# codelibs/ranklib

Measured on AMD Instinct MI355X. Metric: boosting rounds/sec (LambdaMART -ranker 6, NDCG@10), higher is better.
Workload: dtype int64 fixed-point histograms + f64 lambdas/scores (f32 leaf chains as in the Java)

## Files before the change

ranklib_amd/_native.py:

```python
import ctypes as C
import os

import numpy as np

_HERE = os.path.dirname(os.path.abspath(__file__))
LIB_PATH = os.environ.get("RLHIP_LIB") or os.path.join(_HERE, "lib", "librlhip.so")


class RankLibError(RuntimeError):
    """Mirrors ciir.umass.edu.utilities.RankLibError (utilities/RankLibError.java:9-43)."""


class RlParams(C.Structure):
    _fields_ = [("n_trees", C.c_int32), ("n_leaves", C.c_int32), ("n_threshold", C.c_int32),
                ("min_leaf_support", C.c_int32), ("early_stop_rounds", C.c_int32), ("learning_rate", C.c_float),
                ("metric", C.c_int32), ("metric_k", C.c_int32), ("device", C.c_int32), ("flags", C.c_int32),
                ("ranker", C.c_int32), ("feature_sampling_rate", C.c_float), ("seed", C.c_uint64)]


RL_METRIC = dict(NDCG=0, DCG=1, MAP=2, ERR=3, P=4, RR=5)
RL_CA_METRIC = dict(NDCG=0, DCG=1, MAP=2, ERR=3, P=4, RR=5)
RL_NORM_KIND = dict(sum=0, zscore=1, linear=2)
RL_EVAL_METRIC = dict(RL_CA_METRIC, BEST=6)

# ... 581 lines not shown
        need = C.c_int64(0)
        check(lib().rl_model_to_text(self.h, None, 0, C.byref(need)))
        buf = C.create_string_buffer(need.value)
        check(lib().rl_model_to_text(self.h, buf, need.value, C.byref(need)))
        return buf.value.decode("ascii")

    def bin_stride(self):
        s = C.c_int32(0)
        check(lib().rl_bin_stride(self.h, C.byref(s)))
        return s.value

    def quant_exponent(self):
        e = C.c_int32(0)
        check(lib().rl_quant_exponent(self.h, C.byref(e)))
        return e.value

    def hist_features(self):
        n = C.c_int32(0)
        check(lib().rl_hist_features(self.h, C.byref(n), None, 0))
        cols = np.zeros(n.value, np.int32)
        check(lib().rl_hist_features(self.h, C.byref(n), cols.ctypes.data_as(C.POINTER(C.c_int32)), n.value))
        return n.value, cols

    def array(self, name):
        which = ARR[name]
        TS = self.bin_stride()
        F_hist = self.hist_features()[0] if name in ("NBINS", "THRESHOLDS", "BINS", "ROOT_COUNT", "ROOT_SUM", "ROOT_SUM_FIXED", "ROOT_SUM_JAVA") else self.F
        shapes = {
            "LAMBDA": ((self.N,), np.float64), "WEIGHT": ((self.N,), np.float64), "SCORE": ((self.N,), np.float64),
            "VALID_SCORE": ((self.Nv,), np.float64), "NBINS": ((F_hist,), np.int32),
            "THRESHOLDS": ((F_hist, TS), np.float32), "BINS": ((F_hist, self.N), np.uint16),
            "ROOT_COUNT": ((F_hist, TS), np.int32), "ROOT_SUM": ((F_hist, TS), np.float64), "ROOT_SUM_JAVA": ((F_hist, TS), np.float64),
            "QUANT": ((self.N,), np.int64), "ROOT_SUM_FIXED": ((F_hist, TS, 2), np.int64),
            "NDCG_PER_QUERY": ((self.Q,), np.float64), "CHAIN_STATS": ((6,), np.int32), "GROW_STATS": ((4,), np.int32), "GROW_DOCS": ((4,), np.int64), "BUBBLES": ((4,), np.int64), "PIECE_STATS": ((2,), np.int64), "SPARSE_INFO": ((8,), np.int64), "PHASE_CLOCKS": ((64, 32), np.int64), "BLOCK_TRACE": ((64, 3, 2048, 8), np.int64), "STEP_LOG": ((8 + 8 * 8192,), np.int32), "TIE_STATS": ((10,), np.int64), "LAUNCH_ARMS": ((ARM["COUNT_"],), np.int64), "CHAIN_MISS": ((2, self.cap + 1), np.int32),
        }
        shape, dt = shapes[name]
        out = np.zeros(shape, dt)
        check(lib().rl_get_array(self.h, which, out.ctypes.data, out.nbytes))
        return out

    def timing(self, kernel):
        ms, n, b = C.c_double(0), C.c_int64(0), C.c_double(0)
        check(lib().rl_get_timing(self.h, KERNEL[kernel], C.byref(ms), C.byref(n), C.byref(b)))
        return ms.value, n.value, b.value

    def reset_timing(self):
        check(lib().rl_reset_timing(self.h))

    def set_timing_flags(self, flags):
        check(lib().rl_set_timing_flags(self.h, flags))

    def close(self):
        if getattr(self, "h", None) and self.h.value:
            lib().rl_destroy(self.h)
            self.h = C.c_void_p()

    def __del__(self):
        try:
            self.close()
        except Exception:
            pass


MODEL_PATH_NONE, MODEL_PATH_TILED, MODEL_PATH_GENERIC = 0, 1, 2
MODEL_PATH_PERMUTED = 3
PERMUTED_BATCH = 16
MODEL_PATH_COVER, MODEL_PATH_CONTRIBS = 4, 5
# ... 630 lines not shown
```

ranklib_amd/csrc/rl_internal.h:

```cpp
#pragma once
#include <hip/hip_runtime.h>
#include <stdint.h>

#include <string>
#include <vector>

#include "../../include/rlhip.h"

namespace rl {

constexpr int kThreads = 256;
constexpr int kWave = 64;
constexpr int kFinThreads = 320;
constexpr int kLog2Chunk = 14;
constexpr int kChunk = 1 << kLog2Chunk;
#ifndef RL_NODE_CHUNK
#define RL_NODE_CHUNK 8192
#endif
constexpr int kNodeChunk = RL_NODE_CHUNK;
constexpr int kMinChunk = 512;
#ifndef RL_HIST_DOCS
#define RL_HIST_DOCS 2
#endif
constexpr int kHistDocs = RL_HIST_DOCS;
// ... 34 lines not shown
    double  sq_response;
    long long tot_hi; unsigned long long tot_lo;
    long long sq;
    float   output; int32_t gcount;
    int32_t pl, pr;
    int32_t fid;
    int32_t prepared;
    int32_t best_cl, tie;
    unsigned long long ph;
    long long best_hi; unsigned long long best_lo;
};

struct SlotRec {
    int32_t node, left, right, build_left;
    int32_t pstart, pcount, pbuf, f, t;
    int32_t tile0, ntiles;
    int32_t chunk0, nchunks;
    int32_t nleft;
    int32_t cs, skip_hist;
    long long sq_left;
};

struct TreeState {
    int32_t n_nodes, nslots, done, taken;
    int32_t qsize, n_leaves, E, E2;
    int32_t n_splits, error, tiles_total, chunks_total;
    int32_t arrive, epoch, step, tree_seq;
    unsigned long long maxabs_bits;
    long long root_sq;
    int32_t stall_n, stall_node[kSpec], defer_any, stall_pad[2 + (4 - kSpec % 4) % 4];
    SlotRec slot[kSpec];
    int32_t arrive1[kSpec][16];
};

struct TreeSlot {
    int32_t n_nodes, pad;
};

struct FeatBest;
struct Ctx {
    int32_t N, Npad, Q, F, TS, L, MAXN, NC, mls, k, maxChunks, nTiles, FG, numFG;
    float lr;
    int32_t rank, n_ranks;
    int32_t sharded;
    int32_t Nglobal;
    int32_t sub_child;
    int32_t hist_nt;
    int32_t node_div, node_min, node_chunk;
    const int32_t *live_nthr;
    int32_t n_live; const int32_t *live;
    int32_t limb_words;
    const int32_t *fcol;
    int32_t fs_on;
    int32_t fs_size;
    unsigned long long seed;
    int32_t tie_on;
    int32_t mart, metric;
    long long *dist_buf;
    const uint16_t *bins;
    const uint16_t *gbins;
    const uint16_t *dbins;
    int32_t p8, pd_stride;
    const unsigned char *pbins;
    const uint16_t *phib;
    const unsigned char *pdbins;
    const uint8_t *cr_grp;
// ... 108 lines not shown
```

ranklib_amd/csrc/rl_k_ensemble.inc:

```

namespace rl {

struct EnsTree {
    int32_t *feat_idx;
    float *thr;
    int32_t *left, *right;
    float *out;
    int32_t *n_nodes;
    int32_t *count;
    double *deviance;
};

__global__ __launch_bounds__(kThreads) void k_export_tree(const Ctx c, const EnsTree e, int tree)
{
    const TreeState *st = c.st;
    const int nn = st->n_nodes;
    for (int i = threadIdx.x; i < nn; i += kThreads) {
        const NodeRec &X = c.nodes[i];
        if (X.fid < 0) continue;
        const size_t o = (size_t)tree * c.MAXN + X.fid;
        const bool leaf = X.left < 0;
        e.feat_idx[o] = leaf ? -1 : (c.vcol ? c.vcol[X.best_f] : X.best_f);
        e.thr[o] = leaf ? 0.f : c.thr[(size_t)X.best_f * c.TS + X.best_t];
        e.left[o] = leaf ? -1 : c.nodes[X.left].fid; e.right[o] = leaf ? -1 : c.nodes[X.right].fid;
        e.out[o] = leaf ? X.output : 0.f;
        e.count[o] = X.gcount;
        e.deviance[o] = X.deviance;
    }
    if (threadIdx.x == 0) e.n_nodes[tree] = 2 * st->n_splits + 1;
}

__global__ __launch_bounds__(kThreads) void k_valid_update(const EnsTree e, int MAXN, int tree, const float *X, int n, int F,
                                                            float lr, double *vscores)
{
    const size_t o = (size_t)tree * MAXN;
    for (int i = blockIdx.x * kThreads + threadIdx.x; i < n; i += gridDim.x * kThreads) {
        const float *row = X + (size_t)i * F;
        int nd = 0;
        while (e.feat_idx[o + nd] != -1) nd = (row[e.feat_idx[o + nd]] <= e.thr[o + nd]) ? e.left[o + nd] : e.right[o + nd];
        vscores[i] += (double)lr * (double)e.out[o + nd];
    }
}

__global__ __launch_bounds__(kThreads) void k_ensemble_eval(const EnsTree e, int MAXN, int nt, const float *X, int64_t n,
                                                             int stride, float w, float *out, double *out_d)
{
    for (int64_t i = (int64_t)blockIdx.x * kThreads + threadIdx.x; i < n; i += (int64_t)gridDim.x * kThreads) {
        const float *row = X + (size_t)i * stride;
        float s = 0.f;
        for (int t = 0; t < nt; t++) {
            const size_t o = (size_t)t * MAXN;
            int nd = 0;
            while (e.feat_idx[o + nd] != -1) {
                const int fc = e.feat_idx[o + nd];
                const float v = (fc < stride) ? row[fc] : 0.f;
                nd = (v <= e.thr[o + nd]) ? e.left[o + nd] : e.right[o + nd];
            }
            s = (float)((double)s + (double)e.out[o + nd] * (double)w);
        }
        if (out) out[i] = s;
        if (out_d) out_d[i] = (double)s;
    }
// ... 4 lines not shown
```

ranklib_amd/csrc/rl_k_leaf.inc:

```

namespace rl {

constexpr int kLeafTableCap = 1024;

__global__ __launch_bounds__(kThreads) void k_leaf_table(const Ctx c, const ChainBufs cb, int32_t *seg_buf)
{
    __shared__ int s_left[kLeafTableCap], s_right[kLeafTableCap], s_start[kLeafTableCap], s_buf[kLeafTableCap], s_stack[kLeafTableCap];
    TreeState *st = c.st;
    if (threadIdx.x == 0 && c.grow_docs[8] != 0ull) {
        const unsigned long long now = wall_clock64();
        c.grow_docs[4] += now - c.grow_docs[8]; c.grow_docs[5] += 1ull; c.grow_docs[8] = 0ull;
    }
    const int nn = st->n_nodes;
    if (nn <= kLeafTableCap) {
        for (int x = threadIdx.x; x < nn; x += kThreads) {
            const NodeRec &X = c.nodes[x];
            s_left[x] = X.left; s_right[x] = X.right; s_start[x] = X.start; s_buf[x] = X.buf;
        }
        __syncthreads();
        if (threadIdx.x != 0) return;
        int n = 0, sp = 0, tiles = 0, prev = 0;
        s_stack[sp++] = 0;
        while (sp > 0) {
            const int x = s_stack[--sp];
// ... 106 lines not shown
        for (int p = blockIdx.x * kThreads + threadIdx.x; p < N; p += gridDim.x * kThreads) {
            int lo = 0, hi = nl - 1;
            while (lo < hi) { const int mid = (lo + hi + 1) >> 1; if (c.leaf_start[mid] <= p) lo = mid; else hi = mid - 1; }
            const int node = c.leaf_node[lo];
            const NodeRec &X = c.nodes[node];
            const int k = (node == 0) ? p : c.idx[X.buf][p];
            c.scores[k] += (double)c.lr * (double)X.output;
        }
        return;
    }
    constexpr int RUN = kScoreBatch * kThreads;
    for (int base = blockIdx.x * RUN; base < N; base += gridDim.x * RUN) {
        int p[kScoreBatch], k[kScoreBatch]; double step[kScoreBatch], sc[kScoreBatch];
        int buf[kScoreBatch];
#pragma unroll
        for (int u = 0; u < kScoreBatch; u++) {
            p[u] = min(base + u * kThreads + (int)threadIdx.x, N - 1);
            int lo = 0, hi = nl - 1;
            while (lo < hi) { const int mid = (lo + hi + 1) >> 1; if (s_start[mid] <= p[u]) lo = mid; else hi = mid - 1; }
            buf[u] = s_buf[lo]; step[u] = s_step[lo];
        }
#pragma unroll
        for (int u = 0; u < kScoreBatch; u++) k[u] = c.idx[max(buf[u], 0)][p[u]];
#pragma unroll
        for (int u = 0; u < kScoreBatch; u++) { if (buf[u] < 0) k[u] = p[u]; }
#pragma unroll
        for (int u = 0; u < kScoreBatch; u++) sc[u] = c.scores[k[u]];
#pragma unroll
        for (int u = 0; u < kScoreBatch; u++)
            if (base + u * kThreads + (int)threadIdx.x < N) c.scores[k[u]] = sc[u] + step[u];
    }
}

__global__ __launch_bounds__(kThreads) void k_score_stream(const Ctx c)
{
    __shared__ double s_step[1024];
    const TreeState *st = c.st;
    const int nl = st->n_leaves;
    for (int i = threadIdx.x; i < nl; i += kThreads) s_step[i] = (double)c.lr * (double)c.nodes[c.leaf_node[i]].output;
    __syncthreads();
    const int N = c.N;
    constexpr int RUN = kScoreBatch * kThreads;
    for (int base = blockIdx.x * RUN; base < N; base += gridDim.x * RUN) {
        int k[kScoreBatch]; unsigned short lf[kScoreBatch]; double sc[kScoreBatch];
#pragma unroll
        for (int u = 0; u < kScoreBatch; u++) { k[u] = min(base + u * kThreads + (int)threadIdx.x, N - 1); lf[u] = c.leaf_of[k[u]]; sc[u] = c.scores[k[u]]; }
#pragma unroll
        for (int u = 0; u < kScoreBatch; u++)
            if (base + u * kThreads + (int)threadIdx.x < N) c.scores[k[u]] = sc[u] + s_step[min((int)lf[u], 1023)];
    }
}

__global__ __launch_bounds__(64) void k_float_mean(const double *v, int n, float *out)
{
    float s = 0.f;
    for (int base = 0; base < n; base += 64) {
        const int i = base + lane_id();
        const double x = (i < n) ? v[i] : 0.0;
        const uint32_t a0 = (uint32_t)d2bits(x), a1 = (uint32_t)(d2bits(x) >> 32);
        const int m = min(64, n - base);
#pragma unroll
        for (int j = 0; j < 64; j++) {
            if (j < m) {
                const uint64_t ua = ((uint64_t)(uint32_t)__builtin_amdgcn_readlane((int)a1, j) << 32) | (uint32_t)__builtin_amdgcn_readlane((int)a0, j);
                s = float_chain_step(s, bits2d(ua));
            }
        }
    }
    if (lane_id() == 0) *out = s / (float)n;
}

__global__ __launch_bounds__(64) void k_double_mean(const double *v, int n, double *out)
{
    if (threadIdx.x != 0) return;
    double s = 0.0;
    for (int i = 0; i < n; i++) s += v[i];
    *out = s / n;
}

}
```

ranklib_amd/csrc/rl_k_select.inc:

```

namespace rl {

__device__ __forceinline__ void queue_insert_lds(int *q, double *qd, int &qsize, int node, double d)
{
    int i = 0;
    while (i < qsize) { if (qd[i] > d) i++; else break; }
    for (int j = qsize; j > i; j--) { q[j] = q[j - 1]; qd[j] = qd[j - 1]; }
    q[i] = node; qd[i] = d;
    qsize++;
}

__device__ __forceinline__ int node_chunks(const Ctx &c, int cnt) { return cnt <= 0 ? 0 : (cnt + chunk_docs<false>(c, cnt) - 1) / chunk_docs<false>(c, cnt); }

__device__ __forceinline__ void prepare_children(const Ctx &c, NodeRec *N, int p, int l, SlotRec &sl)
{
    NodeRec &P = N[p];
    const int r = l + 1;
    const int cl = P.best_cl;
    const long long thi = P.best_hi; const unsigned long long tlo = P.best_lo;
    NodeRec Lc, Rc;
    Lc.start = P.start; Lc.count = 0; Lc.gcount = cl; Lc.buf = 1 - P.buf; Lc.parent = p; Lc.left = Lc.right = -1;
    Rc.start = P.start; Rc.count = 0; Rc.gcount = P.gcount - cl; Rc.buf = 1 - P.buf; Rc.parent = p; Rc.left = Rc.right = -1;
    const i128 tl = make_i128(thi, tlo);
    const i128 tr = make_i128(P.tot_hi, P.tot_lo) - tl;
// ... 365 lines not shown
    if (tid < nsel) prepare_children(c, N, sel[tid], nn0 + 2 * tid, st.slot[tid]);
    if (c.steplog && tid < nsel) {
        const int e = atomicAdd(&c.steplog[0], 1);
        if (e < kStepLogCap) {
            int *o = c.steplog + 8 + 8 * e; const NodeRec &P = N[sel[tid]];
            o[0] = st.tree_seq; o[1] = 0; o[2] = st.step + 1; o[3] = tid; o[4] = P.gcount; o[5] = st.slot[tid].build_left ? P.best_cl : P.gcount - P.best_cl; o[6] = P.tie; o[7] = nsel;
        }
    }
    __syncthreads();
    if (tid == 0) {
        int tiles = 0, chunks = 0;
        balance_slots(c, st.slot, nsel);
        for (int j = 0; j < nsel; j++) {
            st.slot[j].tile0 = tiles; tiles += st.slot[j].ntiles;
            st.slot[j].chunk0 = chunks; chunks += st.slot[j].nchunks;
        }
        st.tiles_total = tiles; st.chunks_total = chunks;
        st.n_nodes = nn0 + 2 * nsel;
        st.arrive = 0; st.epoch++;
        for (int j = 0; j < kSpec * 16; j++) (&st.arrive1[0][0])[j] = 0;
    }
    __syncthreads();
    RL_CLK(true, 12);
    if (nodes_in_lds) copy_words(c.nodes, N, st.n_nodes * (int)(sizeof(NodeRec) / 8));
    RL_CLK(true, 13);
#ifdef RL_PHASE_CLOCKS
    if (tid == 0 && st.tree_seq == c.trace_tree) c.clk[(st.step & 63) * 32 + 28] = (long long)wall_clock64();
#endif
    if (tid == 0) st.step++;
    __syncthreads();
    copy_words(c.st, &st, sizeof(TreeState) / 8);
    if (tid == 0 && c.progress)
        __hip_atomic_store(c.progress, ((unsigned long long)(unsigned)st.tree_seq << 32) | (st.stall_n > 0 ? (1ull << 31) : 0ull) | (st.defer_any ? (1ull << 30) : 0ull) |
                                           ((unsigned long long)((unsigned)st.step & 0x1fffffffu) << 1) | (st.done ? 1ull : 0ull),
                           __ATOMIC_RELAXED, __HIP_MEMORY_SCOPE_SYSTEM);
}

template <bool WIDE = false>
__device__ __forceinline__ void select_step(const Ctx &c, bool is_root, unsigned char *smem, bool nodes_in_lds, bool dist)
{
    if (nodes_in_lds) select_step_t<true, WIDE>(c, is_root, smem, dist);
    else select_step_t<false, WIDE>(c, is_root, smem, dist);
}

}
```

ranklib_amd/csrc/rl_round.inc:

```

namespace rl {

struct RoundPlan {
    size_t hist_lds, red_lds, par_lds, fin_lds, slot_words;
    int hist_gx, rootCs, rootChunks, nodes_in_lds, jbg, steps;
};

static int round_plan(const rl_trainer *t, RoundPlan &pl)
{
    const Ctx &c = t->ctx;
    pl.hist_lds = (size_t)c.sub * ((c.sub == 16 && c.TS <= kHistLdsStride) ? kHistLdsStride : c.TS) * 12;
    pl.hist_gx = c.numFG * (kHistFG / c.sub);
    pl.red_lds = (size_t)c.TS * 20;
    pl.rootCs = std::min(kChunk, std::max(kMinChunk, (((c.N + 63) / 64 + 255) & ~255)));
    pl.rootChunks = (c.N + pl.rootCs - 1) / pl.rootCs;
    pl.nodes_in_lds = (select_lds_bytes(c.L, c.NC, true, c.F, c.fs_on != 0) <= 60 * 1024) ? 1 : 0;
    pl.par_lds = (c.TS <= kParCacheTS) ? (size_t)c.TS * 20 + 8 : 0;
    pl.fin_lds = std::max((size_t)c.TS * (c.java ? 28 : 20) + 8 + pl.par_lds, select_lds_bytes(c.L, c.NC, pl.nodes_in_lds != 0, c.F, c.fs_on != 0));
    pl.jbg = (c.TS + 63) / 64;
    if (pl.fin_lds > 128 * 1024) return fail(RL_ERR_UNSUPPORTED, "too many features / leaves for the growth bookkeeping in LDS (feature sampling needs 64 bytes per feature)");
    pl.steps = std::max(c.L - 1, 1);
    pl.slot_words = (size_t)c.F * c.TS * c.limb_words + 4;
    return RL_OK;
}

static int enqueue_lambdas(rl_trainer *t, int &n_max)
{
    Ctx &c = t->ctx;
    hipStream_t s = t->stream;
    const int m = t->round;
    RL_HIP(hipMemsetAsync(&c.st->maxabs_bits, 0, sizeof(unsigned long long) + sizeof(long long), s));
    n_max = 0;
    if (c.mart) {
        ScopedTiming tm(t, RL_KERNEL_LAMBDA, (double)c.N * 20.0);
        n_max = std::min(2048, (c.N + kThreads - 1) / kThreads);
        t->arms[RL_ARM_LAM_MART]++;
        hipLaunchKernelGGL(k_mart_residual, dim3(n_max), dim3(kThreads), 0, s, c.labels, (const double *)c.scores, c.lw, c.N, t->d_wmax);
    } else {
        ScopedTiming tm(t, RL_KERNEL_LAMBDA, (double)c.N * 28.0);
        const double *ideal = (c.metric == RL_METRIC_NDCG) ? (m == 0 ? c.ideal0 : c.ideal1) : nullptr;
        LamArgs g{t->tr.d_ss, t->tr.d_sl, t->tr.d_srel, t->tr.d_sidx, c.qoff, t->tr.d_docq, ideal, c.disc,
                  t->d_T, c.lw, &c.st->maxabs_bits, c.N, c.k, c.k, c.metric, t->p.metric_k,
                  t->tr.d_aux_i, t->tr.d_aux_a, t->tr.d_aux_b, t->d_wmax, t->tr.d_ext_rd};
        if (t->d_T == nullptr) {
            const int mode = (c.metric == RL_METRIC_ERR) ? 1 : (c.metric == RL_METRIC_MAP) ? 2 : (c.metric == RL_METRIC_P) ? 3 : (c.metric == RL_METRIC_RR) ? 4 : 0;
            static const int mode_arm[5] = {RL_ARM_LAM_FUSED, RL_ARM_LAM_ERR, RL_ARM_LAM_MAP, -1, -1};
            const bool cp = t->knobs.lam_compact && mode == 0;
            auto lds_of = [&](int bt) { return (size_t)c.k * (bt + 8) * 16 + (size_t)c.k * 24 + lambda_fused_extra_bytes(mode, c.k, bt) + (cp ? lambda_fused_cp_bytes(c.k, bt) : 0); };
            n_max = 0;
            const DataSet &d = t->tr;
            int lam_used = 0;
            RL_HIP(hipEventRecord(t->ev_lam_fork, s));
            auto lam_stream = [&]() -> hipStream_t {
                const int lam_side = t->knobs.lam_side;
                if (lam_used >= lam_side) return s;
                hipStream_t ls = t->lam_s[lam_used++];
                (void)hipStreamWaitEvent(ls, t->ev_lam_fork, 0);
                return ls;
            };
#define RL_LAUNCH_FUSED(BT, cls)                                                                                                             \
            if (d.n_qcls[cls] > 0) {                                                                                                         \
                hipStream_t ls = lam_stream();                                                                                               \
                if (cp) t->arms[RL_ARM_LAM_COMPACT]++; else if (mode_arm[mode] >= 0) t->arms[mode_arm[mode]]++;                               \
                t->arms[ls == s ? RL_ARM_LAM_ON_MAIN : RL_ARM_LAM_ON_SIDE]++;                                                                \
// ... 59 lines not shown
        if (c.sp_on) {
            hipLaunchKernelGGL(k_hist_sp<kHistLdsStride>, dim3(c.sp_ngroups, pl.rootChunks), dim3(kSpThreads), (size_t)kHistFG * kHistLdsStride * 8, s, c, pl.rootCs);
        }
    }
    if (t->dist) {
        hipLaunchKernelGGL(k_hist_reduce, dim3(c.F), dim3(kFinThreads), pl.red_lds, s, c, 1);
        int rcd = t->dist->allreduce(c.dist_buf, (size_t)c.F * c.TS * c.limb_words + 4, DT_I64, OP_SUM, s);
        if (rcd) return rcd;
        hipLaunchKernelGGL((k_hist_finish<true, true>), dim3(c.F), dim3(kFinThreads), pl.fin_lds, s, c, pl.nodes_in_lds);
    } else if (c.java) {
        hipLaunchKernelGGL(k_jgather, dim3((c.N + kPartTile - 1) / kPartTile), dim3(kThreads), 0, s, c, 1);
        if (c.jmap) hipLaunchKernelGGL(k_jhist2, dim3(c.n_live + 1, 1), dim3(kJ2Threads), 0, s, c, 1, c.jmap, c.jinv, c.jone);
        else hipLaunchKernelGGL(k_jhist, dim3(c.n_live, pl.jbg + 2, 1), dim3(64), 0, s, c, 1, pl.jbg);
        hipLaunchKernelGGL((k_hist_finish<true, false, true>), dim3(c.n_live), dim3(kFinThreads), pl.fin_lds, s, c, pl.nodes_in_lds);
    } else if (t->knobs.step2 && c.TS <= kFin2MaxT) {
        hipLaunchKernelGGL(k_fin2_root, dim3(c.n_live), dim3(kFin2RootThreads), 0, s, c, pl.rootChunks);
        hipLaunchKernelGGL(k_select_root, dim3(1), dim3(kFinThreads), pl.fin_lds, s, c, pl.nodes_in_lds);
    } else hipLaunchKernelGGL((k_hist_finish<true, false>), dim3(c.n_live), dim3(kFinThreads), pl.fin_lds, s, c, pl.nodes_in_lds);
    t->tree_seq++;
    return RL_OK;
}

struct Growth {
    int it = 0, extra = 0;
    bool throttle;
    bool saw_end = false;
    bool defer_seen = false;
    explicit Growth(const Ctx &c) : throttle(c.progress != nullptr) {}
};
enum class Next { Go, Again, Ended };

static bool word_stalled(const rl_trainer *t, unsigned long long w) { return t->ctx.tie_on && (w >> 32) == t->tree_seq && ((w >> 31) & 1ull); }
static bool word_finished(const rl_trainer *t, unsigned long long w) { return (w >> 32) == t->tree_seq && (w & 1); }

static int after_stall(rl_trainer *t, const RoundPlan &pl, Growth &g, Next &next)
{
    Ctx &c = t->ctx;
    int rcs = resolve_ties(t, pl.fin_lds, pl.nodes_in_lds);
    if (rcs) return rcs;
    g.extra += 2;
    bool ended, deferred;
    if (c.progress) {
        const unsigned long long w = __atomic_load_n(t->h_progress, __ATOMIC_ACQUIRE);
        if ((w >> 32) != t->tree_seq) return fail(RL_ERR_STATE, "tie-break: the progress word is not this tree's (internal error)");
        ended = (w & 1ull) != 0;
        deferred = ((w >> 30) & 1ull) != 0;
        g.it = (int)((unsigned)(w & 0x3fffffffull) >> 1);
    } else {
        TreeState sth;
        RL_HIP(hipMemcpy(&sth, c.st, sizeof(sth), hipMemcpyDeviceToHost));
        ended = sth.done != 0;
        deferred = sth.defer_any != 0;
        g.it = sth.step;
    }
    if (ended) g.defer_seen = deferred;
    next = ended ? Next::Ended : Next::Again;
    return RL_OK;
}

static int growth_gate(rl_trainer *t, const RoundPlan &pl, Growth &g, Next &next)
{
    Ctx &c = t->ctx;
    hipStream_t s = t->stream;
    next = Next::Go;
    if (g.throttle && c.tie_on && !t->dist) {
        const unsigned long long w0 = __atomic_load_n(t->h_progress, __ATOMIC_ACQUIRE);
        if (word_stalled(t, w0)) return after_stall(t, pl, g, next);
    }
    const int ahead = t->dist ? t->knobs.dist_ahead : t->knobs.step_ahead;
    if (!g.throttle || g.it < ahead) return RL_OK;
    const unsigned long long want = ((unsigned long long)t->tree_seq << 32) | ((unsigned long long)(unsigned)(g.it - ahead) << 1);
    unsigned long long w = __atomic_load_n(t->h_progress, __ATOMIC_ACQUIRE);
    if (t->dist) {
        unsigned spins = 0;
        const auto t0w = std::chrono::steady_clock::now();
        while ((w & ~(3ull << 30)) < want && !word_finished(t, w) && !word_stalled(t, w)) {
            w = __atomic_load_n(t->h_progress, __ATOMIC_ACQUIRE);
            if ((++spins & 0xfffff) == 0) {
                const hipError_t q = hipStreamQuery(s);
                if (q != hipSuccess && q != hipErrorNotReady) return fail(RL_ERR_HIP, std::string("device error while growing a tree: ") + hipGetErrorString(q));
                if (std::chrono::duration<double>(std::chrono::steady_clock::now() - t0w).count() > t->knobs.dist_timeout_s)
                    return fail(RL_ERR_COMM, "timed out after " + std::to_string((int)t->knobs.dist_timeout_s) + " s waiting for growth step " + std::to_string(g.it - ahead) +
                                             " of tree " + std::to_string(t->tree_seq) + " (a rank of the job is missing from a collective?)");
            }
        }
        const int step_w = (int)((unsigned)(w & 0x3fffffffull) >> 1);
        if (word_finished(t, w) && step_w <= g.it - ahead) { g.defer_seen = ((w >> 30) & 1ull) != 0; next = Next::Ended; return RL_OK; }
        if (word_stalled(t, w) && step_w <= g.it - ahead) return after_stall(t, pl, g, next);
    } else {
        const auto behind = [&](unsigned long long v) {
            if ((v >> 32) != t->tree_seq) return true;
            return (unsigned)((v & 0x3fffffffull) >> 1) < (unsigned)(g.it - ahead) && !(v & 1) && !((v >> 31) & 1);
        };
        if (behind(w)) {
            const auto t0 = std::chrono::steady_clock::now();
            unsigned spins = 0;
            while (behind(w = __atomic_load_n(t->h_progress, __ATOMIC_ACQUIRE))) {
                if ((++spins & 1023) == 0 && std::chrono::steady_clock::now() - t0 > std::chrono::milliseconds(200)) { g.throttle = false; break; }
            }
        }
        if (word_stalled(t, w)) next = Next::Again;
        else if (word_finished(t, w)) { g.defer_seen = ((w >> 30) & 1ull) != 0; next = Next::Ended; }
    }
    return RL_OK;
}

static int enqueue_growth_step(rl_trainer *t, const RoundPlan &pl, Growth &g, Next &next)
{
    Ctx &c = t->ctx;
    hipStream_t s = t->stream;
    next = Next::Go;
    if (t->dist && !c.cum_cnt_loc) {
        hipLaunchKernelGGL(k_part_count, dim3(c.nTiles), dim3(kThreads), 0, s, c);
        hipLaunchKernelGGL(k_part_scatter<false>, dim3(c.nTiles), dim3(kThreads), 0, s, c);
    } else hipLaunchKernelGGL(k_part_scatter<true>, dim3(c.nTiles), dim3(kThreads), 0, s, c);
    t->arms[RL_ARM_STEPS_ENQUEUED]++;
    {
        ScopedTiming tm(t, RL_KERNEL_HIST_NODE, 0.0);
        launch_hist<false>(c, t->knobs, t->arms, pl.hist_gx, c.maxChunks, pl.hist_lds, s);
    }
    if (t->dist) {
        hipLaunchKernelGGL(k_hist_reduce, dim3(c.F, kSpec), dim3(kFinThreads), pl.red_lds, s, c, 0);
        const int max_slots = std::min(kSpec, 1 << std::min(g.it, 8));
        int rcd = t->dist->allreduce(c.dist_buf, pl.slot_words * max_slots, DT_I64, OP_SUM, s);
        if (rcd) return rcd;
        const size_t sel2_lds_d = select2_lds_bytes(c.L, c.NC);
        if (t->knobs.step2 && c.TS <= kFin2MaxT && !c.fs_on && c.F <= kSel2MaxF && c.L > 0 && c.L + 2 <= 64 && sel2_lds_d <= 60 * 1024) {
            hipLaunchKernelGGL(k_fin2<true>, dim3(c.F, kSpec), dim3(kFin2Threads), 0, s, c);
            hipLaunchKernelGGL(k_select2<false>, dim3(1), dim3(kSel2Threads), sel2_lds_d, s, c);
        } else hipLaunchKernelGGL((k_hist_finish<false, true>), dim3(c.F, kSpec), dim3(kFinThreads), pl.fin_lds, s, c, pl.nodes_in_lds);
        if (!c.progress && g.it + 1 < pl.steps + g.extra && ((g.it >= 7 && (g.it - 7) % 3 == 0) || c.tie_on)) {
            TreeState sth;
            RL_HIP(hipStreamSynchronize(s));
            RL_HIP(hipMemcpy(&sth, c.st, sizeof(sth), hipMemcpyDeviceToHost));
            if (sth.stall_n > 0) return after_stall(t, pl, g, next);
// ... 48 lines not shown
    Ctx &c = t->ctx;
    hipStream_t s = t->stream;
    hipLaunchKernelGGL(k_leaf_table, dim3(1), dim3(kThreads), 0, s, c, t->leaf_chain, t->d_seg_buf);
    if (t->p.flags & RL_FLAG_SERIAL_CHAIN) {
        hipLaunchKernelGGL(k_leaf_chain, dim3(c.L), dim3(64), 0, s, c);
        return RL_OK;
    }
    if (t->p.flags & RL_FLAG_FAST_LEAF) {
        const FastLeafArgs fa{c.lw, c.idx[0], c.idx[1], t->d_seg_buf, c.leaf_start, &c.st->n_leaves, c.MAXN + 1, stream_scores ? c.leaf_of : nullptr,
                              t->d_fast_part, (int32_t)t->fast_slots, t->d_fast_sums, c.nodes, c.leaf_node, c.mart};
        hipLaunchKernelGGL(k_fast_leaf_tiles, dim3((unsigned)t->fast_slots), dim3(kFastTile), 0, s, fa);
        hipLaunchKernelGGL(k_fast_leaf_finish, dim3((unsigned)(c.MAXN + 1)), dim3(kFastTile), 0, s, fa);
        return RL_OK;
    }
    const ChainSource src{nullptr, nullptr, c.lw, c.idx[0], c.idx[1], t->d_seg_buf, stream_scores ? c.leaf_of : nullptr};
    const ChainBufs *sums = &t->leaf_chain;
    if (t->dist && t->piece_chains) {
        int rcp = enqueue_leaf_chains_pieces(t, src);
        if (rcp) return rcp;
    } else if (t->dist) {
        int rco = enqueue_leaf_chains_owner(t, src);
        if (rco) return rco;
        sums = &t->gchain;
    } else enqueue_chain(t, t->leaf_chain, src);
    hipLaunchKernelGGL(k_leaf_output, dim3((c.L + kThreads - 1) / kThreads), dim3(kThreads), 0, s, c, *sums);
    return RL_OK;
}

static int enqueue_scores_and_metrics(rl_trainer *t, bool stream_scores)
{
    Ctx &c = t->ctx;
    hipStream_t s = t->stream;
    const int m = t->round;
    if (stream_scores) hipLaunchKernelGGL(k_score_stream, dim3(std::max(1, std::min(2048, (c.N + kScoreBatch * kThreads - 1) / (kScoreBatch * kThreads)))), dim3(kThreads), 0, s, c);
    else hipLaunchKernelGGL(k_score_update, dim3(std::max(1, std::min(4096, (c.N + kScoreBatch * kThreads - 1) / (kScoreBatch * kThreads)))), dim3(kThreads), 0, s, c);
    hipLaunchKernelGGL(k_export_tree, dim3(1), dim3(kThreads), 0, s, c, t->ens, m);
    RL_HIP(hipGetLastError());
    const bool use_side = !t->has_valid;
    if (use_side && t->side_pending) RL_HIP(hipStreamWaitEvent(s, t->ev_metric, 0));
    int rc = launch_rank(t, t->tr, c.scores, t->tr.d_ndcg, true);
    if (rc != RL_OK) return rc;
    if (use_side) {
        const double *mq = t->tr.d_ndcg; int mQ = t->tr.Q;
        if (t->dist) { rc = gather_queries(t, t->tr.d_ndcg, &mq); if (rc != RL_OK) return rc; mQ = t->Qglobal; }
        RL_HIP(hipEventRecord(t->ev_ranked, s));
        RL_HIP(hipStreamWaitEvent(t->side, t->ev_ranked, 0));
        enqueue_metric_mean(t, mq, mQ, c.round_metric + 2 * (size_t)m, t->side);
        RL_HIP(hipEventRecord(t->ev_metric, t->side));
        t->side_pending = true;
    } else if (t->dist) {
        const double *gq = nullptr;
        rc = gather_queries(t, t->tr.d_ndcg, &gq);
        if (rc != RL_OK) return rc;
        enqueue_metric_mean(t, gq, t->Qglobal, c.round_metric + 2 * (size_t)m);
    } else enqueue_metric_mean(t, t->tr.d_ndcg, t->tr.Q, c.round_metric + 2 * (size_t)m);
    if (t->has_valid) {
        hipLaunchKernelGGL(k_valid_update, dim3(std::min<int64_t>(4096, (t->va.N + kThreads - 1) / kThreads)), dim3(kThreads), 0, s,
                           t->ens, c.MAXN, m, (const float *)t->va.d_X, (int)t->va.N, t->F, c.lr, t->va.d_scores);
        rc = launch_rank(t, t->va, t->va.d_scores, t->va.d_ndcg, false);
        if (rc != RL_OK) return rc;
        if (t->dist) {
            const double *gq = nullptr;
            rc = gather_queries(t, t->va.d_ndcg, &gq, true);
            if (rc != RL_OK) return rc;
            enqueue_metric_mean(t, gq, t->vQglobal, c.round_metric + 2 * (size_t)m + 1);
        } else enqueue_metric_mean(t, t->va.d_ndcg, t->va.Q, c.round_metric + 2 * (size_t)m + 1);
    }
    RL_HIP(hipGetLastError());
    t->round = m + 1;
// ... 34 lines not shown
```

ranklib_amd/csrc/rl_step2.inc:

```

namespace rl {

constexpr int kFin2Threads = 320;
constexpr int kFin2Waves = kFin2Threads / 64;
constexpr int kFin2MaxT = kFin2Threads;

struct Fin2WaveRec { double S; int t, c, flags; };

template <bool DIST = false>
__global__ __launch_bounds__(kFin2Threads) void k_fin2(const Ctx c)
{
    const TreeState *st = c.st;
    RL_TR_BEGIN();
    const int slot = blockIdx.y;
    const int st_done = st->done, st_nslots = st->nslots, E = st->E;
    const SlotRec sl = st->slot[slot];
    const int f = (!DIST && c.live) ? c.live[blockIdx.x] : (int)blockIdx.x;
    const int TS = c.TS, T = (!DIST && c.live) ? c.live_nthr[blockIdx.x] : c.nthr[f];
    if (st_done || slot >= st_nslots) return;
    const bool sq_block = blockIdx.x == 0;
    if (sl.skip_hist && !sq_block) return;
    const int tid = threadIdx.x, lane = tid & 63, wave = tid >> 6;
    const int nodeP = sl.node, nodeB = sl.build_left ? sl.left : sl.right, nodeS = sl.build_left ? sl.right : sl.left, sideB = sl.build_left ? 0 : 1;
    const int ch0 = sl.chunk0;
// ... 602 lines not shown
        }
        __builtin_amdgcn_fence(__ATOMIC_ACQ_REL, "workgroup");
        __builtin_amdgcn_wave_barrier();
        if (lane == 0) {
            if (nsel == 1 && budget == 1 && c.skip_last) {
                SlotRec &s0 = st.slot[0];
                s0.skip_hist = 1; s0.nchunks = 0;
                atomicAdd(&c.grow_docs[0], (unsigned long long)(-(long long)(s0.build_left ? s0.nleft : s0.pcount - s0.nleft)));
            }
            int tiles = 0, chunks = 0;
            if (!(nsel == 1 && st.slot[0].skip_hist)) balance_slots(c, st.slot, nsel);
            for (int j = 0; j < nsel; j++) {
                st.slot[j].tile0 = tiles; tiles += st.slot[j].ntiles;
                st.slot[j].chunk0 = chunks; chunks += st.slot[j].nchunks;
            }
            st.tiles_total = tiles; st.chunks_total = chunks;
            st.n_nodes = nn0 + 2 * nsel;
            st.arrive = 0; st.epoch++;
#ifdef RL_PHASE_CLOCKS
            if (st.tree_seq == c.trace_tree) {
                long long *o_ = c.clk + (st.step & 63) * 32;
                const long long t5_ = strict_clock();
                o_[20] = tk_[0]; o_[21] = tk_[1]; o_[22] = tk_[2]; o_[23] = tk_[3]; o_[24] = tk_[4]; o_[25] = t5_; o_[28] = t5_;
            }
#endif
            st.step++;
        }
    }
    __syncthreads();
    {
        const int nw = st.n_nodes * kNodeW;
        for (int i = tid; i < nw; i += kSel2Threads) ((unsigned long long *)c.nodes)[i] = ((const unsigned long long *)N)[i];
        if (tid < kStW) ((unsigned long long *)c.st)[tid] = ((const unsigned long long *)&st)[tid];
        if (tid == 0 && c.progress)
            __hip_atomic_store(c.progress, ((unsigned long long)(unsigned)st.tree_seq << 32) | (st.stall_n > 0 ? (1ull << 31) : 0ull) | (st.defer_any ? (1ull << 30) : 0ull) |
                                               ((unsigned long long)((unsigned)st.step & 0x1fffffffu) << 1) | (st.done ? 1ull : 0ull),
                               __ATOMIC_RELAXED, __HIP_MEMORY_SCOPE_SYSTEM);
    }
}

}
```

ranklib_amd/csrc/rl_trainer.hip:

```cpp
#include <algorithm>
#include <chrono>
#include <cmath>
#include <limits>
#include <cstdio>
#include <cstring>
#include <map>
#include <memory>

#include "rl_internal.h"
#include "rl_lists_host.h"
#include "rl_knobs.h"
#include "rl_device.h"
#include "rl_wave.h"
#include "rl_kernels_init.inc"
#include "rl_chain.inc"
#include "rl_kernels_round.inc"
#include "rl_fast_leaf.inc"
#include "rl_step2.inc"
#include "rl_java_order.inc"
#include "rl_csc.inc"
#include "rl_tie.inc"
#include "rl_membench.inc"
#include "rl_dist.inc"
#include "rl_model.h"
// ... 14 lines not shown
    int32_t *d_aux_i = nullptr; double *d_aux_a = nullptr, *d_aux_b = nullptr;
    int32_t *d_ext_rd = nullptr;
    int32_t *d_qsmall = nullptr, *d_qbig = nullptr, *d_qtiny = nullptr; int32_t n_small = 0, n_big = 0, n_tiny = 0, max_big = 0, n_small_long = 0; bool all_small = false;
    int32_t *d_qhuge = nullptr, *d_relscratch = nullptr; int32_t n_huge = 0;
    int32_t *d_qcls[5] = {nullptr, nullptr, nullptr, nullptr, nullptr}; int32_t n_qcls[5] = {0, 0, 0, 0, 0};
};

struct TimingSlot { double ms = 0; int64_t launches = 0; double bytes = 0; };

}

using namespace rl;

struct rl_trainer {
    rl_params p;
    Knobs knobs;
    int32_t F = 0;
    std::vector<int32_t> feature_ids;
    std::vector<int32_t> vcol;
    DataSet tr, va;
    bool has_train = false, has_valid = false, inited = false, finished = false;
    hipStream_t stream = nullptr;
    hipStream_t side = nullptr; hipEvent_t ev_ranked = nullptr, ev_metric = nullptr; bool side_pending = false;
    hipStream_t lam_s[3] = {nullptr, nullptr, nullptr}; hipEvent_t ev_lam_fork = nullptr, ev_lam_join[3] = {nullptr, nullptr, nullptr};
    DevPool pool;
    Ctx ctx;
    EnsTree ens;
    int32_t L_eff = 0;
    int32_t *d_tie_flag = nullptr;
    int64_t sp_entries = 0; int32_t sp_cols = 0;
    int32_t cr_groups = 0; double cr_entries = 0, cr_overflow = 0;
    double err_max = 16.0;
    int32_t round = 0;
    int64_t arms[RL_ARM_COUNT_] = {};
    unsigned long long *h_progress = nullptr; uint32_t tree_seq = 0;
    unsigned long long chain_seq = 0; std::vector<void *> pinned;
    int32_t synced_rounds = 0;
    long long tie_stalls = 0, tie_nodes = 0, tie_chain_nodes = 0, tie_chain_docs = 0;
    long long tie_batches = 0;
    bool fin_split = false;
    long long tie_phase_us[6] = {0, 0, 0, 0, 0, 0};
    long long chain_calls[2] = {0, 0}, chain_repairs[2] = {0, 0}, chain_timeouts = 0, chain_wait_us = 0;
    long long tie_regrown = 0;
    long long tie_us = 0, tie_spec_segs = 0, tie_spec_miss = 0, tie_spec_serial = 0, tie_spec_repairs = 0;
    std::vector<int32_t> h_nthr; std::vector<char> tie_blob;
    void *tie_pin = nullptr; size_t tie_pin_cap = 0;
    void *tie_buf = nullptr; size_t tie_cap = 0, tie_hint = 0;
    int32_t n_kept = 0;
    int32_t best_round = 2147483647 - 2;
    double best_score = 0.0;
    std::vector<float> h_metrics;
    std::vector<HostTree> trees;
    float *d_final_f = nullptr; double *d_final_d = nullptr, *d_mean = nullptr;
    ChainBufs leaf_chain, metric_chain;
    int32_t *d_seg_buf = nullptr;
    double2 *d_fast_part = nullptr, *d_fast_sums = nullptr; int64_t fast_slots = 0;
    double2 *d_T = nullptr;
    double *d_wmax = nullptr;
    float *d_vmetric = nullptr;
    std::vector<std::pair<hipEvent_t, hipEvent_t>> ev_pending[RL_KERNEL_COUNT_];
    std::vector<double> ev_bytes[RL_KERNEL_COUNT_];
    std::vector<hipEvent_t> ev_free;
    TimingSlot timing[RL_KERNEL_COUNT_];
    int32_t rank = 0, n_ranks = 1;
    std::unique_ptr<DistBackend> dist;
    std::vector<int32_t> all_N, all_Q;
    int64_t Nglobal = 0; int32_t Qglobal = 0, Qmax = 0;
    ChainBufs gchain;
// ... 713 lines not shown

int rl_quant_exponent(const rl_trainer *t, int32_t *e)
{
    if (check_trainer(t)) return RL_ERR_INVALID;
    if (!t->inited) return fail(RL_ERR_STATE, "rl_init has not been called");
    TreeState st;
    RL_HIP(hipMemcpy(&st, t->ctx.st, sizeof(st), hipMemcpyDeviceToHost));
    if (e) *e = st.E;
    return RL_OK;
}

int rl_get_array(rl_trainer *t, int32_t which, void *out, int64_t cap_bytes)
{
    if (check_trainer(t)) return RL_ERR_INVALID;
    if (!t->inited) return fail(RL_ERR_STATE, "rl_init has not been called");
    RL_HIP(hipSetDevice(t->p.device));
    RL_HIP(hipStreamSynchronize(t->stream));
    const Ctx &c = t->ctx;
    const void *src = nullptr; size_t bytes = 0;
    switch (which) {
    case RL_ARR_LAMBDA: case RL_ARR_WEIGHT: {
        bytes = (size_t)c.N * 8;
        if ((int64_t)bytes > cap_bytes) return fail(RL_ERR_INVALID, "output buffer too small");
        RL_HIP(hipMemcpy2D(out, 8, (const char *)c.lw + (which == RL_ARR_WEIGHT ? 8 : 0), 16, 8, (size_t)c.N, hipMemcpyDeviceToHost));
        return RL_OK;
    }
    case RL_ARR_SCORE: src = c.scores; bytes = (size_t)c.N * 8; break;
    case RL_ARR_VALID_SCORE: if (!t->has_valid) return fail(RL_ERR_STATE, "no validation set"); src = t->va.d_scores; bytes = (size_t)t->va.N * 8; break;
    case RL_ARR_NBINS: src = c.nthr; bytes = (size_t)c.F * 4; break;
    case RL_ARR_THRESHOLDS: src = c.thr; bytes = (size_t)c.F * c.TS * 4; break;
    case RL_ARR_ROOT_COUNT: src = c.cum_cnt; bytes = (size_t)c.F * c.TS * 4; break;
    case RL_ARR_QUANT: src = c.q; bytes = (size_t)c.N * 8; break;
    case RL_ARR_NDCG_PER_QUERY: src = c.ndcg_q; bytes = (size_t)c.Q * 8; break;
    case RL_ARR_GROW_STATS: src = c.grow_stats; bytes = 16; break;
    case RL_ARR_GROW_DOCS: src = c.grow_docs; bytes = 32; break;
    case RL_ARR_BUBBLES: src = c.grow_docs + 4; bytes = 32; break;
    case RL_ARR_PIECE_STATS: {
        const int64_t v[2] = {t->piece_rounds, t->piece_misses};
        if ((int64_t)sizeof(v) > cap_bytes) return fail(RL_ERR_INVALID, "output buffer too small");
        memcpy(out, v, sizeof(v));
        return RL_OK;
    }
    case RL_ARR_SPARSE_INFO: {
        const int64_t v[8] = {c.sp_on ? c.sp_ngroups : 0, t->sp_entries, c.sp_on ? c.numFG - c.sp_ngroups : c.numFG, t->sp_cols,
                              c.crows ? t->cr_groups : 0, (int64_t)t->cr_entries, (int64_t)t->cr_overflow, c.cr_stride};
        if (cap_bytes < (int64_t)sizeof(v)) return fail(RL_ERR_INVALID, "output buffer too small");
        memcpy(out, v, sizeof(v));
        return RL_OK;
    }
    case RL_ARR_LAUNCH_ARMS: {
        int64_t v[RL_ARM_COUNT_];
        memcpy(v, t->arms, sizeof(v));
        v[RL_ARM_SET_STEP_AHEAD] = t->knobs.step_ahead; v[RL_ARM_SET_DIST_AHEAD] = t->knobs.dist_ahead;
        v[RL_ARM_SET_P8] = c.p8; v[RL_ARM_SET_DM_ROOT] = c.dm_root; v[RL_ARM_SET_DM_DIV] = c.dm_div; v[RL_ARM_SET_SUB_CHILD] = c.sub_child; v[RL_ARM_SET_HIST_NT] = c.hist_nt;
        v[RL_ARM_SET_ANY_RUNS] = c.any_runs; v[RL_ARM_SET_CROWS] = c.crows ? 1 : 0; v[RL_ARM_SET_TIE_ON] = c.tie_on; v[RL_ARM_SET_NODE_DIV] = c.node_div;
        v[RL_ARM_SET_NODE_MIN] = c.node_min; v[RL_ARM_SET_BALANCE] = c.balance; v[RL_ARM_SET_BALANCE_TARGET] = c.balance_target; v[RL_ARM_SET_BALANCE_MIN] = c.balance_min;
        v[RL_ARM_SET_BALANCE_CAP] = c.balance_cap; v[RL_ARM_SET_NODE_CHUNK] = c.node_chunk; v[RL_ARM_SET_MAX_CHUNKS] = c.maxChunks;
        if (cap_bytes < (int64_t)(RL_ARM_REPLAY_TILED * sizeof(int64_t))) return fail(RL_ERR_INVALID, "output buffer too small");
        memcpy(out, v, std::min<size_t>(sizeof(v), (size_t)cap_bytes));
        return RL_OK;
    }
    case RL_ARR_TIE_STATS: {
        const int64_t v[10] = {t->tie_stalls, t->tie_nodes, t->tie_chain_nodes, t->tie_chain_docs, t->tie_us, t->tie_spec_segs, t->tie_spec_miss, t->tie_spec_serial,
                                t->tie_batches, t->tie_regrown};
        if (cap_bytes < (int64_t)sizeof(v)) return fail(RL_ERR_INVALID, "output buffer too small");
        memcpy(out, v, sizeof(v));
        return RL_OK;
// ... 95 lines not shown
```

Measured before the change: 368.3.

## Fuse score update with tree export and signal last split early to the host

Merges the score-stream and tree-export kernels into one launch. Block 0 exports the tree and zeroes the per-round scalars, which removes a separate kernel launch and the next round's memset. It also adds a 'last next' bit to the device progress word, set when the only remaining slot skips its histogram, so the host growth loop can decide the tree has ended one step earlier. To make room for that bit, the step field shrinks to 28 bits, and a new counter is exposed through GROW_STATS.

```diff
diff --git a/ranklib_amd/_native.py b/ranklib_amd/_native.py
--- a/ranklib_amd/_native.py
+++ b/ranklib_amd/_native.py
@@ -637,7 +637,7 @@
             "THRESHOLDS": ((F_hist, TS), np.float32), "BINS": ((F_hist, self.N), np.uint16),
             "ROOT_COUNT": ((F_hist, TS), np.int32), "ROOT_SUM": ((F_hist, TS), np.float64), "ROOT_SUM_JAVA": ((F_hist, TS), np.float64),
             "QUANT": ((self.N,), np.int64), "ROOT_SUM_FIXED": ((F_hist, TS, 2), np.int64),
-            "NDCG_PER_QUERY": ((self.Q,), np.float64), "CHAIN_STATS": ((6,), np.int32), "GROW_STATS": ((4,), np.int32), "GROW_DOCS": ((4,), np.int64), "BUBBLES": ((4,), np.int64), "PIECE_STATS": ((2,), np.int64), "SPARSE_INFO": ((8,), np.int64), "PHASE_CLOCKS": ((64, 32), np.int64), "BLOCK_TRACE": ((64, 3, 2048, 8), np.int64), "STEP_LOG": ((8 + 8 * 8192,), np.int32), "TIE_STATS": ((10,), np.int64), "LAUNCH_ARMS": ((ARM["COUNT_"],), np.int64), "CHAIN_MISS": ((2, self.cap + 1), np.int32),
+            "NDCG_PER_QUERY": ((self.Q,), np.float64), "CHAIN_STATS": ((6,), np.int32), "GROW_STATS": ((5,), np.int32), "GROW_DOCS": ((4,), np.int64), "BUBBLES": ((4,), np.int64), "PIECE_STATS": ((2,), np.int64), "SPARSE_INFO": ((8,), np.int64), "PHASE_CLOCKS": ((64, 32), np.int64), "BLOCK_TRACE": ((64, 3, 2048, 8), np.int64), "STEP_LOG": ((8 + 8 * 8192,), np.int32), "TIE_STATS": ((10,), np.int64), "LAUNCH_ARMS": ((ARM["COUNT_"],), np.int64), "CHAIN_MISS": ((2, self.cap + 1), np.int32),
         }
         shape, dt = shapes[name]
         out = np.zeros(shape, dt)
diff --git a/ranklib_amd/csrc/rl_internal.h b/ranklib_amd/csrc/rl_internal.h
--- a/ranklib_amd/csrc/rl_internal.h
+++ b/ranklib_amd/csrc/rl_internal.h
@@ -90,6 +90,9 @@
     SlotRec slot[kSpec];
     int32_t arrive1[kSpec][16];
 };
+
+constexpr unsigned long long kProgressLastNext = 1ull << 29;
+constexpr unsigned long long kProgressStepMask = 0x1fffffffull;
 
 struct TreeSlot {
     int32_t n_nodes, pad;
diff --git a/ranklib_amd/csrc/rl_k_ensemble.inc b/ranklib_amd/csrc/rl_k_ensemble.inc
--- a/ranklib_amd/csrc/rl_k_ensemble.inc
+++ b/ranklib_amd/csrc/rl_k_ensemble.inc
@@ -11,7 +11,7 @@
     double *deviance;
 };
 
-__global__ __launch_bounds__(kThreads) void k_export_tree(const Ctx c, const EnsTree e, int tree)
+__device__ __forceinline__ void export_tree_block(const Ctx &c, const EnsTree &e, int tree)
 {
     const TreeState *st = c.st;
     const int nn = st->n_nodes;
@@ -28,6 +28,18 @@
         e.deviance[o] = X.deviance;
     }
     if (threadIdx.x == 0) e.n_nodes[tree] = 2 * st->n_splits + 1;
+}
+
+__global__ __launch_bounds__(kThreads) void k_export_tree(const Ctx c, const EnsTree e, int tree) { export_tree_block(c, e, tree); }
+
+__global__ __launch_bounds__(kThreads) void k_score_export(const Ctx c, const EnsTree e, int tree)
+{
+    if (blockIdx.x == 0) {
+        export_tree_block(c, e, tree);
+        if (threadIdx.x == 0) { c.st->maxabs_bits = 0ull; c.st->root_sq = 0ll; }
+        return;
+    }
+    score_stream_block(c, (int)blockIdx.x - 1, (int)gridDim.x - 1);
 }
 
 __global__ __launch_bounds__(kThreads) void k_valid_update(const EnsTree e, int MAXN, int tree, const float *X, int n, int F,
diff --git a/ranklib_amd/csrc/rl_k_leaf.inc b/ranklib_amd/csrc/rl_k_leaf.inc
--- a/ranklib_amd/csrc/rl_k_leaf.inc
+++ b/ranklib_amd/csrc/rl_k_leaf.inc
@@ -162,7 +162,7 @@
     }
 }
 
-__global__ __launch_bounds__(kThreads) void k_score_stream(const Ctx c)
+__device__ __forceinline__ void score_stream_block(const Ctx &c, int bid, int nb)
 {
     __shared__ double s_step[1024];
     const TreeState *st = c.st;
@@ -171,7 +171,7 @@
     __syncthreads();
     const int N = c.N;
     constexpr int RUN = kScoreBatch * kThreads;
-    for (int base = blockIdx.x * RUN; base < N; base += gridDim.x * RUN) {
+    for (int base = bid * RUN; base < N; base += nb * RUN) {
         int k[kScoreBatch]; unsigned short lf[kScoreBatch]; double sc[kScoreBatch];
 #pragma unroll
         for (int u = 0; u < kScoreBatch; u++) { k[u] = min(base + u * kThreads + (int)threadIdx.x, N - 1); lf[u] = c.leaf_of[k[u]]; sc[u] = c.scores[k[u]]; }
@@ -180,6 +180,8 @@
             if (base + u * kThreads + (int)threadIdx.x < N) c.scores[k[u]] = sc[u] + s_step[min((int)lf[u], 1023)];
     }
 }
+
+__global__ __launch_bounds__(kThreads) void k_score_stream(const Ctx c) { score_stream_block(c, (int)blockIdx.x, (int)gridDim.x); }
 
 __global__ __launch_bounds__(64) void k_float_mean(const double *v, int n, float *out)
 {
diff --git a/ranklib_amd/csrc/rl_k_select.inc b/ranklib_amd/csrc/rl_k_select.inc
--- a/ranklib_amd/csrc/rl_k_select.inc
+++ b/ranklib_amd/csrc/rl_k_select.inc
@@ -421,7 +421,7 @@
     copy_words(c.st, &st, sizeof(TreeState) / 8);
     if (tid == 0 && c.progress)
         __hip_atomic_store(c.progress, ((unsigned long long)(unsigned)st.tree_seq << 32) | (st.stall_n > 0 ? (1ull << 31) : 0ull) | (st.defer_any ? (1ull << 30) : 0ull) |
-                                           ((unsigned long long)((unsigned)st.step & 0x1fffffffu) << 1) | (st.done ? 1ull : 0ull),
+                                           ((unsigned long long)((unsigned)st.step & 0x0fffffffu) << 1) | (st.done ? 1ull : 0ull),
                            __ATOMIC_RELAXED, __HIP_MEMORY_SCOPE_SYSTEM);
 }
 
diff --git a/ranklib_amd/csrc/rl_round.inc b/ranklib_amd/csrc/rl_round.inc
--- a/ranklib_amd/csrc/rl_round.inc
+++ b/ranklib_amd/csrc/rl_round.inc
@@ -29,7 +29,8 @@
     Ctx &c = t->ctx;
     hipStream_t s = t->stream;
     const int m = t->round;
-    RL_HIP(hipMemsetAsync(&c.st->maxabs_bits, 0, sizeof(unsigned long long) + sizeof(long long), s));
+    if (!t->round_scalars_zeroed) RL_HIP(hipMemsetAsync(&c.st->maxabs_bits, 0, sizeof(unsigned long long) + sizeof(long long), s));
+    t->round_scalars_zeroed = false;
     n_max = 0;
     if (c.mart) {
         ScopedTiming tm(t, RL_KERNEL_LAMBDA, (double)c.N * 20.0);
@@ -155,6 +156,8 @@
 
 static bool word_stalled(const rl_trainer *t, unsigned long long w) { return t->ctx.tie_on && (w >> 32) == t->tree_seq && ((w >> 31) & 1ull); }
 static bool word_finished(const rl_trainer *t, unsigned long long w) { return (w >> 32) == t->tree_seq && (w & 1); }
+static int word_step(unsigned long long w) { return (int)((unsigned)(w & kProgressStepMask) >> 1); }
+static bool word_last_next(const rl_trainer *t, unsigned long long w) { return (w >> 32) == t->tree_seq && (w & kProgressLastNext) != 0; }
 
 static int after_stall(rl_trainer *t, const RoundPlan &pl, Growth &g, Next &next)
 {
@@ -168,7 +171,7 @@
         if ((w >> 32) != t->tree_seq) return fail(RL_ERR_STATE, "tie-break: the progress word is not this tree's (internal error)");
         ended = (w & 1ull) != 0;
         deferred = ((w >> 30) & 1ull) != 0;
-        g.it = (int)((unsigned)(w & 0x3fffffffull) >> 1);
+        g.it = word_step(w);
     } else {
         TreeState sth;
         RL_HIP(hipMemcpy(&sth, c.st, sizeof(sth), hipMemcpyDeviceToHost));
@@ -207,13 +210,13 @@
                                              " of tree " + std::to_string(t->tree_seq) + " (a rank of the job is missing from a collective?)");
             }
         }
-        const int step_w = (int)((unsigned)(w & 0x3fffffffull) >> 1);
+        const int step_w = word_step(w);
         if (word_finished(t, w) && step_w <= g.it - ahead) { g.defer_seen = ((w >> 30) & 1ull) != 0; next = Next::Ended; return RL_OK; }
         if (word_stalled(t, w) && step_w <= g.it - ahead) return after_stall(t, pl, g, next);
     } else {
         const auto behind = [&](unsigned long long v) {
             if ((v >> 32) != t->tree_seq) return true;
-            return (unsigned)((v & 0x3fffffffull) >> 1) < (unsigned)(g.it - ahead) && !(v & 1) && !((v >> 31) & 1);
+            return word_step(v) < g.it - ahead && !(v & 1) && !((v >> 31) & 1);
         };
         if (behind(w)) {
             const auto t0 = std::chrono::steady_clock::now();
@@ -224,6 +227,10 @@
         }
         if (word_stalled(t, w)) next = Next::Again;
         else if (word_finished(t, w)) { g.defer_seen = ((w >> 30) & 1ull) != 0; next = Next::Ended; }
+        else if (word_last_next(t, w) && word_step(w) < g.it) {
+            t->ends_announced++;
+            g.defer_seen = ((w >> 30) & 1ull) != 0; next = Next::Ended;
+        }
     }
     return RL_OK;
 }
@@ -338,9 +345,15 @@
     Ctx &c = t->ctx;
     hipStream_t s = t->stream;
     const int m = t->round;
-    if (stream_scores) hipLaunchKernelGGL(k_score_stream, dim3(std::max(1, std::min(2048, (c.N + kScoreBatch * kThreads - 1) / (kScoreBatch * kThreads)))), dim3(kThreads), 0, s, c);
-    else hipLaunchKernelGGL(k_score_update, dim3(std::max(1, std::min(4096, (c.N + kScoreBatch * kThreads - 1) / (kScoreBatch * kThreads)))), dim3(kThreads), 0, s, c);
-    hipLaunchKernelGGL(k_export_tree, dim3(1), dim3(kThreads), 0, s, c, t->ens, m);
+    const int stream_blocks = std::max(1, std::min(2048, (c.N + kScoreBatch * kThreads - 1) / (kScoreBatch * kThreads)));
+    if (stream_scores && !t->dist && !c.java) {
+        hipLaunchKernelGGL(k_score_export, dim3(stream_blocks + 1), dim3(kThreads), 0, s, c, t->ens, m);
+        t->round_scalars_zeroed = true;
+    } else {
+        if (stream_scores) hipLaunchKernelGGL(k_score_stream, dim3(stream_blocks), dim3(kThreads), 0, s, c);
+        else hipLaunchKernelGGL(k_score_update, dim3(std::max(1, std::min(4096, (c.N + kScoreBatch * kThreads - 1) / (kScoreBatch * kThreads)))), dim3(kThreads), 0, s, c);
+        hipLaunchKernelGGL(k_export_tree, dim3(1), dim3(kThreads), 0, s, c, t->ens, m);
+    }
     RL_HIP(hipGetLastError());
     const bool use_side = !t->has_valid;
     if (use_side && t->side_pending) RL_HIP(hipStreamWaitEvent(s, t->ev_metric, 0));
diff --git a/ranklib_amd/csrc/rl_step2.inc b/ranklib_amd/csrc/rl_step2.inc
--- a/ranklib_amd/csrc/rl_step2.inc
+++ b/ranklib_amd/csrc/rl_step2.inc
@@ -658,11 +658,13 @@
         const int nw = st.n_nodes * kNodeW;
         for (int i = tid; i < nw; i += kSel2Threads) ((unsigned long long *)c.nodes)[i] = ((const unsigned long long *)N)[i];
         if (tid < kStW) ((unsigned long long *)c.st)[tid] = ((const unsigned long long *)&st)[tid];
-        if (tid == 0 && c.progress)
+        if (tid == 0 && c.progress) {
+            const bool last_next = !st.done && st.stall_n == 0 && st.nslots == 1 && st.slot[0].skip_hist != 0;
             __hip_atomic_store(c.progress, ((unsigned long long)(unsigned)st.tree_seq << 32) | (st.stall_n > 0 ? (1ull << 31) : 0ull) | (st.defer_any ? (1ull << 30) : 0ull) |
-                                               ((unsigned long long)((unsigned)st.step & 0x1fffffffu) << 1) | (st.done ? 1ull : 0ull),
+                                               (last_next ? kProgressLastNext : 0ull) | ((unsigned long long)((unsigned)st.step & 0x0fffffffu) << 1) | (st.done ? 1ull : 0ull),
                                __ATOMIC_RELAXED, __HIP_MEMORY_SCOPE_SYSTEM);
-    }
-}
-
-}
+        }
+    }
+}
+
+}
diff --git a/ranklib_amd/csrc/rl_trainer.hip b/ranklib_amd/csrc/rl_trainer.hip
--- a/ranklib_amd/csrc/rl_trainer.hip
+++ b/ranklib_amd/csrc/rl_trainer.hip
@@ -70,8 +70,10 @@
     int32_t cr_groups = 0; double cr_entries = 0, cr_overflow = 0;
     double err_max = 16.0;
     int32_t round = 0;
+    bool round_scalars_zeroed = false;
     int64_t arms[RL_ARM_COUNT_] = {};
     unsigned long long *h_progress = nullptr; uint32_t tree_seq = 0;
+    int64_t ends_announced = 0;
     unsigned long long chain_seq = 0; std::vector<void *> pinned;
     int32_t synced_rounds = 0;
     long long tie_stalls = 0, tie_nodes = 0, tie_chain_nodes = 0, tie_chain_docs = 0;
@@ -851,7 +853,12 @@
     case RL_ARR_ROOT_COUNT: src = c.cum_cnt; bytes = (size_t)c.F * c.TS * 4; break;
     case RL_ARR_QUANT: src = c.q; bytes = (size_t)c.N * 8; break;
     case RL_ARR_NDCG_PER_QUERY: src = c.ndcg_q; bytes = (size_t)c.Q * 8; break;
-    case RL_ARR_GROW_STATS: src = c.grow_stats; bytes = 16; break;
+    case RL_ARR_GROW_STATS: {
+        if (cap_bytes < 16) return fail(RL_ERR_INVALID, "output buffer too small");
+        RL_HIP(hipMemcpy(out, c.grow_stats, 16, hipMemcpyDeviceToHost));
+        if (cap_bytes >= 20) ((int32_t *)out)[4] = (int32_t)t->ends_announced;
+        return RL_OK;
+    }
     case RL_ARR_GROW_DOCS: src = c.grow_docs; bytes = 32; break;
     case RL_ARR_BUBBLES: src = c.grow_docs + 4; bytes = 32; break;
     case RL_ARR_PIECE_STATS: {
```

Result: no change. 368.2 (-0.0%).
